# mlhenderson/cori-intml-examples

Hardware: AMD Instinct MI355X
Metric: images/sec (whole node) RPV CNN training (higher is better)
Workload: dtype bf16; 1 GPU; model=RPV CNN conv[16,32,64] fc[128] 64x64x3 (DistTrain_rpv), global_batch=128, per_gpu_batch=128, optimizer=Adam, parallelism=dp1, steps_per_graph=32

## Files before the change

### cori_intml_examples_amd/csrc/kernels/args.h

```cpp
#pragma once
#include "common.h"

struct BwdThrough {
  const bf16* prev_out = nullptr;
  const uint8_t* prev_code = nullptr;
  int prev_relu = 0, prev_pool = 0;
  int pH = 1, pW = 1, pC = 0, pCs = 0;
  int cH = 1, cW = 1;
  uint32_t drop_thr = 0;
  float drop_scale = 1.f;
  uint32_t seed = 0, stream_id = 0;
  bf16* dy = nullptr;
  int wt = 0;
};

struct PackRoute {
  int lo, hi, kind;
  int KHW, Cin, Cout, Cs, Csb;
  int NT, NTb;
  long long fwd, bwd;
};
#define MAX_ROUTES 8

struct OptimArgs {
// ... 145 lines not shown
  int spec = 1;
  int fix = 1;
};

struct WgradArgs {
  const bf16* x = nullptr;
  int B = 0, H = 0, W = 0, Cs_in = 0;
  int Ho = 0, Wo = 0, KH = 1, KW = 1, stride = 1, pad_t = 0, pad_l = 0;
  int Ktiles = 0;
  const bf16* dy = nullptr;
  int Cs_dy = 0;
  int NT = 0;
  int P = 0;
  int px_per_split = 0;
  int KT = 0;
  float* slab = nullptr;
  float* bslab = nullptr;
  int R = 1, blocks_per_split = 1;
  const uint8_t* dy_code = nullptr;
  int dHp = 0, dWp = 0;
  const bf16* zero = nullptr;
  int dbg = 0;
  unsigned long long* ts = nullptr;
  unsigned long long* ts2 = nullptr;
  OptimArgs opt;
  int opt_w = -1, opt_b = -1;
  int opt_nograd = 0;
  int spec = 1;
  long long pk_fwd = -1, pk_bwd = -1;
  int pk_NT = 0, pk_NTb = 0;
  int wt = 0;
  int xpix = 0, xrow = 0, dyld = 0;
  int kperm = 0;
  const int* xidx = nullptr;
  const StepState* xst = nullptr;
};

#define WG_GEO_INTS(F)                                                                                       \
  F(H) F(W) F(Cs_in) F(Ho) F(Wo) F(KH) F(KW) F(stride) F(pad_t) F(pad_l) F(Ktiles) F(NT) F(Cs_dy) F(dHp) F(dWp) \
  F(R) F(xpix) F(xrow) F(dyld) F(kperm) F(wt)

struct StepBeginArgs {
  StepState* st = nullptr;
  int training = 1;
  int bs = 0;
  int opt_kind = 0;
  float beta1 = 0.9f, beta2 = 0.999f, decay = 0.f, schedule_decay = 0.004f;
};

struct DenseFwdArgs {
  const bf16* x = nullptr;
  int M = 0, Ks = 0;
  const bf16* wpk = nullptr;
  int NT = 0, KS = 0;
  int splits = 1, ks_per_split = 0;
  float* part = nullptr;
  int mode = 0;
  const StepState* st = nullptr;
  BwdThrough bt;
  int book = 0;
  StepBeginArgs sb;
};

struct DenseEpiArgs {
  const float* part = nullptr;
  int splits = 1, M = 0, N = 0, Ns = 0, ldp = 0;
  const float* bias = nullptr;
  int relu = 0;
  bf16* out = nullptr;
// ... 246 lines not shown
```

### cori_intml_examples_amd/csrc/kernels/bindings.cpp

```cpp
#include <algorithm>
#include <pybind11/pybind11.h>
#include <pybind11/stl.h>

#include "args.h"

namespace py = pybind11;

void launch_conv_halo(const ConvMMArgs& a, int ntc, hipStream_t s);
size_t conv_halo_lds_bytes(const ConvMMArgs& a, int ntc);
void launch_conv_tile(const ConvMMArgs& a, int ntc, hipStream_t s, bool big, int nbuf);
bool launch_conv_hs(const ConvMMArgs& a, int ntc, hipStream_t s, int nwv, int order);
bool conv_hs_ok(const ConvMMArgs& a, int ntc, int nwv);
long long conv_tile_big_blocks(const ConvMMArgs& a, int ntc);
size_t conv_tile_lds_bytes(int ntc);
void launch_wgrad_tile(const WgradArgs& a, int ntc, hipStream_t s);
size_t wgrad_tile_lds_bytes(int ntc);
void launch_wgrad_halo(const WgradArgs& a, int MT, int NTT, int splits, hipStream_t s);
size_t wgrad_halo_lds_bytes(const WgradArgs& a, int MT, int NTT);
int wgrad_halo_resident(const WgradArgs& a, int MT, int NTT, bool bias);
int wgrad_halo_variant(const WgradArgs& a, int MT, int NTT);
int dual_halo_variant(const ConvMMArgs& ca, int ntc, const WgradArgs& wa, int MT, int NTT, bool xp, bool extras);
bool dual_halo_dgrad_fixed(const ConvMMArgs& ca, int ntc, const WgradArgs& wa, int MT, int NTT, bool xp, bool extras);
int head_rows_per_block(bool fused);
int head_epi_max();
void launch_wgrad(const WgradArgs& a, int ktw, int ntt, int splits, hipStream_t s);
size_t wgrad_lds_bytes(int KT, int NTT);
void launch_dense_fwd(const DenseFwdArgs& a, hipStream_t s);
void launch_dense_epi(const DenseEpiArgs& a, hipStream_t s);
int dense_groups(int M, int NT, int KS);
bool dense_big(int NT, int KS);
void launch_head(const HeadArgs& a, hipStream_t s);
bool launch_dual_halo(const ConvMMArgs& ca, int ntc, const WgradArgs& wa, int MT, int NTT, int splits,
                      const DualExtra& x, hipStream_t s);
bool launch_dense_bwd_dual(const WgradArgs& wa, int ktw, int ntt, int splits, const DenseFwdArgs& da,
                           hipStream_t s);
void launch_dense_wgrad(const WgradArgs& a, int kg, int ntt, int splits, hipStream_t s, int order, bool late);
size_t dense_wgrad_lds_bytes(int kg, int ntt);
void launch_dense_dx(const DenseFwdArgs& a, int ntc, hipStream_t s);
void launch_dense_bwd_pair(const WgradArgs& wa, int kg, int ntt, int splits, const DenseFwdArgs& da, int ntc,
                           hipStream_t s);
void launch_conv_stack_fwd(const ConvStackArgs& a, hipStream_t s);
void launch_init_params(const InitArgs& a, hipStream_t s);
void launch_synth(const SynthArgs& a, hipStream_t s);
int conv_stack_threads();
int conv_stack_variant(const ConvStackArgs& a);
bool conv_stack_fixed(const ConvStackArgs& a);
int conv_stack_tabn();
void launch_prologue(const PrologueArgs& a, const PackTable& tab, hipStream_t s);
int gather_gx(int R);
void launch_slab_reduce(float* grad, int lo, int hi, const RedTable& tab, hipStream_t s);
void launch_reduce_optim_end(float* grad, const RedTable& tc, const OptimArgs& a, const XgmiPush& xc,
                             const RedTable& te, const XgmiPush& xe, hipStream_t s);
void launch_reduce_optim(float* grad, const RedTable& tab, const OptimArgs& a, hipStream_t s,
                         const XgmiPush* xp = nullptr);
void launch_optim(const OptimArgs& a, const PackTable& tab, hipStream_t s);
// ... 67 lines not shown
  m.doc() = "cori_intml_examples_amd gfx950 HIP kernels";

  py::class_<BwdThrough>(m, "BwdThrough")
      .def(py::init<>())
      PTR(BwdThrough, prev_out) PTR(BwdThrough, prev_code) RW(BwdThrough, prev_relu)
      RW(BwdThrough, prev_pool) RW(BwdThrough, pH) RW(BwdThrough, pW) RW(BwdThrough, pC)
      RW(BwdThrough, pCs) RW(BwdThrough, cH) RW(BwdThrough, cW) RW(BwdThrough, drop_thr)
      RW(BwdThrough, drop_scale) RW(BwdThrough, seed) RW(BwdThrough, stream_id) PTR(BwdThrough, dy) RW(BwdThrough, wt);

  py::class_<ConvMMArgs>(m, "ConvMMArgs")
      .def(py::init<>())
      PTR(ConvMMArgs, x) RW(ConvMMArgs, B) RW(ConvMMArgs, H) RW(ConvMMArgs, W) RW(ConvMMArgs, Cs_in)
      RW(ConvMMArgs, Ho) RW(ConvMMArgs, Wo) RW(ConvMMArgs, KH) RW(ConvMMArgs, KW) RW(ConvMMArgs, stride)
      RW(ConvMMArgs, pad_t) RW(ConvMMArgs, pad_l) RW(ConvMMArgs, in_dil) RW(ConvMMArgs, KS)
      PTR(ConvMMArgs, wpk) RW(ConvMMArgs, NT) PTR(ConvMMArgs, bias) RW(ConvMMArgs, N) RW(ConvMMArgs, mode)
      RW(ConvMMArgs, flat_out) RW(ConvMMArgs, relu) RW(ConvMMArgs, pool) PTR(ConvMMArgs, out)
      RW(ConvMMArgs, Cs_out) RW(ConvMMArgs, Hp) RW(ConvMMArgs, Wp) PTR(ConvMMArgs, code)
      RW(ConvMMArgs, drop_thr) RW(ConvMMArgs, drop_scale) RW(ConvMMArgs, seed) RW(ConvMMArgs, stream_id)
      PTR(ConvMMArgs, st) RW(ConvMMArgs, bt) RW(ConvMMArgs, R) PTR(ConvMMArgs, in_code) PTR(ConvMMArgs, zero)
      RW(ConvMMArgs, in_pH) RW(ConvMMArgs, in_pW) RW(ConvMMArgs, dbg) PTR(ConvMMArgs, ts) RW(ConvMMArgs, xpix) RW(ConvMMArgs, kpipe) RW(ConvMMArgs, tm)
      RW(ConvMMArgs, spec);

  py::class_<WgradArgs>(m, "WgradArgs")
      .def(py::init<>())
      PTR(WgradArgs, x) RW(WgradArgs, B) RW(WgradArgs, H) RW(WgradArgs, W) RW(WgradArgs, Cs_in)
      RW(WgradArgs, Ho) RW(WgradArgs, Wo) RW(WgradArgs, KH) RW(WgradArgs, KW) RW(WgradArgs, stride)
      RW(WgradArgs, pad_t) RW(WgradArgs, pad_l) RW(WgradArgs, Ktiles) PTR(WgradArgs, dy)
      RW(WgradArgs, Cs_dy) RW(WgradArgs, NT) RW(WgradArgs, P) RW(WgradArgs, px_per_split)
      RW(WgradArgs, KT) PTR(WgradArgs, slab) PTR(WgradArgs, bslab) RW(WgradArgs, R)
      RW(WgradArgs, blocks_per_split) PTR(WgradArgs, dy_code) PTR(WgradArgs, zero) RW(WgradArgs, dHp) RW(WgradArgs, dWp)
      RW(WgradArgs, dbg) PTR(WgradArgs, ts) PTR(WgradArgs, ts2) RW(WgradArgs, opt) RW(WgradArgs, opt_w)
      RW(WgradArgs, opt_b) RW(WgradArgs, xpix) RW(WgradArgs, xrow) RW(WgradArgs, dyld) RW(WgradArgs, kperm)
      PTR(WgradArgs, xidx) PTR(WgradArgs, xst) RW(WgradArgs, pk_fwd) RW(WgradArgs, pk_bwd) RW(WgradArgs, pk_NT)
      RW(WgradArgs, pk_NTb) RW(WgradArgs, wt) RW(WgradArgs, opt_nograd) RW(WgradArgs, spec);

  py::class_<DenseFwdArgs>(m, "DenseFwdArgs")
      .def(py::init<>())
      PTR(DenseFwdArgs, x) RW(DenseFwdArgs, M) RW(DenseFwdArgs, Ks) PTR(DenseFwdArgs, wpk)
      RW(DenseFwdArgs, NT) RW(DenseFwdArgs, KS) RW(DenseFwdArgs, splits) RW(DenseFwdArgs, ks_per_split)
      PTR(DenseFwdArgs, part) RW(DenseFwdArgs, mode) PTR(DenseFwdArgs, st) RW(DenseFwdArgs, bt)
      RW(DenseFwdArgs, book) RW(DenseFwdArgs, sb);

  py::class_<DenseEpiArgs>(m, "DenseEpiArgs")
      .def(py::init<>())
      PTR(DenseEpiArgs, part) RW(DenseEpiArgs, splits) RW(DenseEpiArgs, M) RW(DenseEpiArgs, N)
      RW(DenseEpiArgs, Ns) RW(DenseEpiArgs, ldp) PTR(DenseEpiArgs, bias) RW(DenseEpiArgs, relu)
      PTR(DenseEpiArgs, out) RW(DenseEpiArgs, drop_thr) RW(DenseEpiArgs, drop_scale)
      RW(DenseEpiArgs, seed) RW(DenseEpiArgs, stream_id) PTR(DenseEpiArgs, st);

  py::class_<HeadArgs>(m, "HeadArgs")
      .def(py::init<>())
      PTR(HeadArgs, h) RW(HeadArgs, M) RW(HeadArgs, K) RW(HeadArgs, Ks) RW(HeadArgs, N)
      RW(HeadArgs, flat_C) RW(HeadArgs, flat_Cs) PTR(HeadArgs, w) PTR(HeadArgs, bias) PTR(HeadArgs, y)
      RW(HeadArgs, act) RW(HeadArgs, training) RW(HeadArgs, inv_bs) PTR(HeadArgs, st) PTR(HeadArgs, probs)
      PTR(HeadArgs, wslab) PTR(HeadArgs, bslab) RW(HeadArgs, bt) RW(HeadArgs, epi) PTR(HeadArgs, ts)
      PTR(HeadArgs, yidx) RW(HeadArgs, generic) PTR(HeadArgs, wb);


  py::class_<GatherArgs>(m, "GatherArgs")
      .def(py::init<>())
      PTR(GatherArgs, xs) PTR(GatherArgs, ys) PTR(GatherArgs, perm) PTR(GatherArgs, st)
      RW(GatherArgs, bs) RW(GatherArgs, R) RW(GatherArgs, C) RW(GatherArgs, Nd) PTR(GatherArgs, xb)
      PTR(GatherArgs, yb) RW(GatherArgs, skip_x) PTR(GatherArgs, wb);

  py::class_<StepBeginArgs>(m, "StepBeginArgs")
      .def(py::init<>())
      PTR(StepBeginArgs, st) RW(StepBeginArgs, training) RW(StepBeginArgs, bs) RW(StepBeginArgs, opt_kind)
// ... 141 lines not shown
        const int epb = d.vec4 ? 1024 / d.tpe : 256 / d.tpe;
        t.nblocks += (numel + epb - 1) / epb;
      }, py::arg("slab"), py::arg("stride_s"), py::arg("S"), py::arg("ld"), py::arg("dst_off"), py::arg("numel"),
      py::arg("type"), py::arg("KH"), py::arg("KW"), py::arg("Cin"), py::arg("Cout"), py::arg("Cs"), py::arg("tpe") = -1);

  m.attr("STEP_STATE_BYTES") = (int)sizeof(StepState);
  m.def("set_red_lanes", [](int n) {
    if (n < 1 || n > 256) throw std::invalid_argument("red_lanes: 1..256");
    g_red_lanes = n;
  });
  static_assert(sizeof(PackRoute) == 56 && offsetof(PackRoute, fwd) == 40, "PackRoute layout (models/plan routes)");
  m.attr("PACK_ROUTE_BYTES") = (int)sizeof(PackRoute);
  m.attr("MAX_ROUTES") = MAX_ROUTES;
  m.attr("MAX_RED") = MAX_RED;
  m.attr("STEP_STATE_METRICS_OFFSET") = (int)offsetof(StepState, metric_slots);
  m.attr("STEP_STATE_METRIC_SLOTS") = 16;
  m.attr("STEP_STATE_MSCHED_OFFSET") = (int)offsetof(StepState, m_schedule);
  m.attr("STEP_STATE_LR_OFFSET") = (int)offsetof(StepState, lr);
  m.attr("STEP_STATE_S_OFFSET") = (int)offsetof(StepState, s);
  m.attr("STEP_STATE_WARM_OFFSET") = (int)offsetof(StepState, warm_t0);
  m.attr("STEP_STATE_DATA_OFFSET") = (int)offsetof(StepState, data_x);
  m.attr("STEP_STATE_DATAN_OFFSET") = (int)offsetof(StepState, data_n);
  m.attr("STEP_STATE_DATAW_OFFSET") = (int)offsetof(StepState, data_w);

  m.def("wgrad_lds_bytes", &wgrad_lds_bytes);
  m.def("conv_halo_lds_bytes", &conv_halo_lds_bytes);
  m.def("wgrad_halo_lds_bytes", &wgrad_halo_lds_bytes);
  m.def("wgrad_halo_resident", &wgrad_halo_resident);
  m.def("wgrad_halo_variant", &wgrad_halo_variant);
  m.def("dual_halo_variant", &dual_halo_variant, py::arg("ca"), py::arg("ntc"), py::arg("wa"), py::arg("MT"),
        py::arg("NTT"), py::arg("xp") = false, py::arg("extras") = false);
  m.def("dual_halo_dgrad_fixed", &dual_halo_dgrad_fixed, py::arg("ca"), py::arg("ntc"), py::arg("wa"), py::arg("MT"),
        py::arg("NTT"), py::arg("xp") = false, py::arg("extras") = false);
  m.def("head_rows_per_block", &head_rows_per_block, py::arg("fused") = false);
  m.def("conv_tile_lds_bytes", &conv_tile_lds_bytes);
  m.def("conv_tile", [](const ConvMMArgs& a, int ntc, uintptr_t s, bool big, int nbuf) {
    launch_conv_tile(a, ntc, S(s), big, nbuf); check_last("conv_tile"); }, py::arg("a"), py::arg("ntc"), py::arg("s"),
    py::arg("big") = false, py::arg("nbuf") = 4);
  m.def("conv_tile_big_blocks", &conv_tile_big_blocks);
  m.def("conv_hs_ok", &conv_hs_ok, py::arg("a"), py::arg("ntc"), py::arg("nwv") = 8);
  m.def("conv_hs", [](const ConvMMArgs& a, int ntc, uintptr_t s, int nwv, int order) {
    const bool ok = launch_conv_hs(a, ntc, S(s), nwv, order); check_last("conv_hs"); return ok; },
    py::arg("a"), py::arg("ntc"), py::arg("s"), py::arg("nwv") = 8, py::arg("order") = 0,
    "halo-staged wide conv (stride 1 or the parity classes of a strided dgrad, whole-row blocks of "
    "32 * nwv rows); false (nothing launched) for other shapes");
  m.def("wgrad_tile_lds_bytes", &wgrad_tile_lds_bytes);
  m.def("wgrad_tile", [](const WgradArgs& a, int ntc, uintptr_t s) {
    launch_wgrad_tile(a, ntc, S(s)); check_last("wgrad_tile"); });
  m.def("conv_halo", [](const ConvMMArgs& a, int ntc, uintptr_t s) {
    launch_conv_halo(a, ntc, S(s)); check_last("conv_halo"); });
  m.def("wgrad_halo", [](const WgradArgs& a, int MT, int NTT, int splits, uintptr_t s) {
    launch_wgrad_halo(a, MT, NTT, splits, S(s)); check_last("wgrad_halo"); });
  m.def("wgrad", [](const WgradArgs& a, int ktw, int ntt, int splits, uintptr_t s) {
    launch_wgrad(a, ktw, ntt, splits, S(s)); check_last("wgrad"); });
  m.def("dense_fwd", [](const DenseFwdArgs& a, uintptr_t s) { launch_dense_fwd(a, S(s)); check_last("dense_fwd"); });
  m.def("dense_groups", &dense_groups, "work items per K-split of dense_fwd for (M, NT, KS)");
  m.def("dense_big", &dense_big, "dense_fwd uses the large-weight LDS path for (NT, KS)");
  m.def("dense_epi", [](const DenseEpiArgs& a, uintptr_t s) { launch_dense_epi(a, S(s)); check_last("dense_epi"); });
  m.def("head", [](const HeadArgs& a, uintptr_t s) { launch_head(a, S(s)); check_last("head"); });
  m.def("prologue", [](const PrologueArgs& a, const PackTable& t, uintptr_t s) {
    launch_prologue(a, t, S(s)); check_last("prologue"); });
  m.def("gather_gx", &gather_gx);
  m.def("head_epi_max", &head_epi_max);
  m.def("reduce_optim_end", [](uintptr_t grad, const RedTable& tc, const OptimArgs& a, uintptr_t s,
                               const XgmiPush& xc, const RedTable& te, const XgmiPush& xe) {
    if (!xc.on || !xe.on || xc.mode != 3 || xe.mode != 5) throw std::invalid_argument("reduce_optim_end: modes 3 + 5");
// ... 224 lines not shown
```

### cori_intml_examples_amd/csrc/kernels/wgrad_halo.hip

```cpp

#include <algorithm>
#include <cstdlib>

#include "wgrad_halo_body.h"
#include "wgrad_sig.h"

template <int MTW, int NTT, bool CS4, bool PIPE, bool INSTR>
__global__ __launch_bounds__(256) void wgrad_halo_kernel(const WgradArgs a, const int MT) {
  extern __shared__ __attribute__((aligned(16))) char smem[];
  const size_t lin = blockIdx.x + (size_t)gridDim.x * (blockIdx.y + (size_t)gridDim.y * blockIdx.z);
  if (INSTR && a.ts && threadIdx.x == 0) a.ts[2 * lin] = wall_clock64();
  wgrad_halo_body<MTW, NTT, CS4, PIPE, INSTR>(a, MT, blockIdx.x, blockIdx.y, blockIdx.z, smem);
  if (INSTR && a.ts) {
    __syncthreads();
    if (threadIdx.x == 0) a.ts[2 * lin + 1] = wall_clock64();
  }
}

static bool wh_instr(const WgradArgs& a) { return a.dbg || a.ts || a.ts2; }

size_t wgrad_halo_lds_bytes(const WgradArgs& a, int MT, int NTT) {
  const int W_in = (a.Wo - 1) * a.stride + a.KW;
  const int R_in = (a.R - 1) * a.stride + a.KH;
  const int XP = a.xpix ? a.xpix : a.Cs_in, XR = a.xrow ? a.xrow : W_in;
  const int ldb = a.dyld ? a.dyld : NTT * 16 + 8;
  const size_t x_elems = (size_t)(((R_in * XR * XP) + 7) & ~7);
  const size_t npb32 = (size_t)((a.R * a.Wo + 31) & ~31);
  return std::max<size_t>(x_elems * 2 + npb32 * ldb * 2 + 128 + (size_t)(MT * 4 + 4) * 4, 4 * 16 * WH_SQ * 4);
}

template <int MTW, int NTT, bool CS4>
static void wh_t(const WgradArgs& a, int MT, dim3 grid, size_t lds, hipStream_t s) {
  const bool pipe = grid.x * grid.y * grid.z < 512 && a.blocks_per_split > 1;
  auto k = wh_instr(a) ? (pipe ? wgrad_halo_kernel<MTW, NTT, CS4, true, true> : wgrad_halo_kernel<MTW, NTT, CS4, false, true>)
                       : (pipe ? wgrad_halo_kernel<MTW, NTT, CS4, true, false> : wgrad_halo_kernel<MTW, NTT, CS4, false, false>);
  if (lds > 65536) (void)hipFuncSetAttribute((const void*)k, hipFuncAttributeMaxDynamicSharedMemorySize, (int)lds);
  hipLaunchKernelGGL(k, grid, dim3(256), lds, s, a, MT);
}

int wgrad_halo_variant(const WgradArgs& a, int MT, int NTT) {
  if (!a.spec || wh_instr(a)) return 0;
  const int v = wgrad_sig_find(a, MT, NTT);
  return v && wgrad_sig_at(v).alone ? v : 0;
}

void launch_wgrad_halo(const WgradArgs& a, int MT, int NTT, int splits, hipStream_t s) {
  const bool cs4 = a.Cs_in == 4;
  dim3 grid(splits, (a.NT + NTT - 1) / NTT, (a.Ktiles + MT - 1) / MT);
  const size_t lds = wgrad_halo_lds_bytes(a, MT, NTT);
  if (const int v = wgrad_halo_variant(a, MT, NTT)) {
    wgrad_sig_at(v).alone(a, grid, lds, grid.x * grid.y * grid.z < 512 && a.blocks_per_split > 1, s);
    return;
  }
  const int mtw = (MT + (a.bslab ? 1 : 0) + 3) / 4;
#define C(M_, N_)                                            \
  if (mtw <= M_ && NTT == N_) {                              \
    if (cs4) wh_t<M_, N_, true>(a, MT, grid, lds, s);     \
    else wh_t<M_, N_, false>(a, MT, grid, lds, s);        \
    return;                                                  \
  }
  C(1, 1) C(2, 1) C(4, 1) C(1, 2) C(2, 2) C(4, 2) C(1, 4) C(2, 4) C(4, 4) C(1, 8) C(2, 8)
#undef C
}

int wgrad_halo_resident(const WgradArgs& a, int MT, int NTT, bool bias) {
  const bool cs4 = a.Cs_in == 4;
  const size_t lds = wgrad_halo_lds_bytes(a, MT, NTT);
  const int mtw = (MT + (bias ? 1 : 0) + 3) / 4;
  const void* k = nullptr;
  const bool in = wh_instr(a);
#define C(M_, N_)                                                                                       \
  if (!k && mtw <= M_ && NTT == N_)                                                                     \
    k = cs4 ? (in ? (const void*)wgrad_halo_kernel<M_, N_, true, false, true>                           \
                  : (const void*)wgrad_halo_kernel<M_, N_, true, false, false>)                         \
            : (in ? (const void*)wgrad_halo_kernel<M_, N_, false, false, true>                          \
                  : (const void*)wgrad_halo_kernel<M_, N_, false, false, false>);
  C(1, 1) C(2, 1) C(4, 1) C(1, 2) C(2, 2) C(4, 2) C(1, 4) C(2, 4) C(4, 4) C(1, 8) C(2, 8)
#undef C
  if (!k) return 0;
  int dev = 0, per_cu = 0;
  hipDeviceProp_t prop;
  if (hipGetDevice(&dev) != hipSuccess || hipGetDeviceProperties(&prop, dev) != hipSuccess) return 0;
  if (lds > 65536) (void)hipFuncSetAttribute(k, hipFuncAttributeMaxDynamicSharedMemorySize, (int)lds);
  if (hipOccupancyMaxActiveBlocksPerMultiprocessor(&per_cu, k, 256, lds) != hipSuccess) return 0;
// ... 3 lines not shown
```

### cori_intml_examples_amd/csrc/kernels/wgrad_halo_body.h

```cpp
#pragma once
#include "bwd_through.h"

struct XChunk4 { bf16x4 v; int o; };
struct XChunk8 { bf16x8 v; int o; };

__device__ __forceinline__ bf16x4 tr_read_h(const bf16* p) {
  return __builtin_amdgcn_ds_read_tr16_b64_v4bf16(LDS_PTR(bf16x4, p));
}

#define WH_STAMP(i)                                                                     \
  if (INSTR && a.ts2 && threadIdx.x == 0 && (i) < 16) a.ts2[(size_t)blockIdx.x * 16 + (i)] = wall_clock64();

struct WgGeoRt {
#define F(n) \
  __device__ __forceinline__ static int n(const WgradArgs& a) { return a.n; }
  WG_GEO_INTS(F)
#undef F
  __device__ __forceinline__ static int MT(int mt_launch) { return mt_launch; }
  __device__ __forceinline__ static bool pooled(const WgradArgs& a) { return a.dy_code != nullptr; }
  __device__ __forceinline__ static bool bias(const WgradArgs& a) { return a.bslab != nullptr; }
  __device__ __forceinline__ static bool xidx(const WgradArgs& a) { return a.xidx != nullptr; }
};
template <class S, bool XIDX>
struct WgGeoFix {
#define F(n) \
  __device__ __forceinline__ static constexpr int n(const WgradArgs&) { return S::n; }
  WG_GEO_INTS(F)
#undef F
  __device__ __forceinline__ static constexpr int MT(int) { return S::MT; }
  __device__ __forceinline__ static constexpr bool pooled(const WgradArgs&) { return S::pooled; }
  __device__ __forceinline__ static constexpr bool bias(const WgradArgs&) { return S::bias; }
  __device__ __forceinline__ static constexpr bool xidx(const WgradArgs&) { return XIDX; }
};

template <class G>
__device__ __forceinline__ const bf16* wg_xbase(const WgradArgs& a, int b) {
  if (G::xidx(a)) return reinterpret_cast<const bf16*>(a.xst->data_x) + (size_t)a.xidx[b] * a.xst->data_R;
  return a.x + (size_t)b * G::H(a) * G::W(a) * G::Cs_in(a);
}

#define WH_SQ 20

template <int MTW, int NTT, bool CS4, bool PIPE, bool INSTR = true, class G = WgGeoRt>
__device__ __forceinline__ void wgrad_halo_body(const WgradArgs& a, const int MT_launch, const int bx, const int by,
                                                const int bz, char* smem) {
  const int MT = G::MT(MT_launch);
  const int dbg = INSTR ? a.dbg : 0;
  const int R = G::R(a), s = G::stride(a), Cs = G::Cs_in(a);
  const int W_in = (G::Wo(a) - 1) * s + G::KW(a);
  const int R_in = (R - 1) * s + G::KH(a);
  const int npb = R * G::Wo(a);
  const int npb32 = (npb + 31) & ~31;
  const int XP = G::xpix(a) ? G::xpix(a) : Cs, XR = G::xrow(a) ? G::xrow(a) : W_in;
  const int ldb = G::dyld(a) ? G::dyld(a) : NTT * 16 + 8;
  bf16* xl = reinterpret_cast<bf16*>(smem);
  const int x_elems = ((R_in * XR * XP) + 7) & ~7;
  bf16* dyl = xl + x_elems;
  bf16* zl = dyl + (size_t)npb32 * ldb;
  bf16* ol = zl + 32;
  int* ktab = reinterpret_cast<int*>(zl + 64);

  const int tid = threadIdx.x, wave = __builtin_amdgcn_readfirstlane(tid >> 6), lane = tid & 63, i = lane & 15,
            g = lane >> 4;
  const int mt0 = bz * MT;
  const int nt0 = by * NTT;
  const int KHW = G::KH(a) * G::KW(a);
  const bool do_bias = G::bias(a) && bz == 0;
  const int MTb = MT + (do_bias ? 1 : 0);

  WH_STAMP(0);
  if (tid < 32) reinterpret_cast<uint32_t*>(zl)[tid] = tid < 16 ? 0u : 0x3F803F80u;
  for (int c = tid; c < MT * 4; c += 256) {
    const int k = (mt0 + c / 4) * 16 + 4 * (c & 3);
    const int tap = k / Cs;
    int e = -1;
    if (tap < KHW && mt0 + c / 4 < G::Ktiles(a)) {
// ... 101 lines not shown
          off0 = ((y0 * s) * XR + (q0 - y0 * G::Wo(a)) * s) * XP;
          off1 = ((y1 * s) * XR + (q1 - y1 * G::Wo(a)) * s) * XP;
        }
        const bf16* pbrow = dyl + (size_t)P0 * ldb + 4 * (i & 3);
  #pragma unroll
        for (int v = 0; v < NTT; ++v) {
          const bf16* pb = pbrow + v * 16;
          bfr[v] = __builtin_shufflevector(tr_read_h(pb), tr_read_h(pb + (P1 - P0) * ldb), 0, 1, 2, 3, 4, 5, 6, 7);
        }
  #pragma unroll
        for (int u = 0; u < MTW; ++u) {
          const bf16* pz = u == ubias ? ol : zl;
          const bf16* pa0 = ko[u] >= 0 ? xl + off0 + ko[u] : pz;
          const bf16* pa1 = ko[u] >= 0 ? xl + off1 + ko[u] : pz;
          afr[u] = __builtin_shufflevector(tr_read_h(pa0), tr_read_h(pa1), 0, 1, 2, 3, 4, 5, 6, 7);
        }
      };
      auto mmas = [&](const bf16x8 (&afr)[MTW], const bf16x8 (&bfr)[NTT]) {
  #pragma unroll
        for (int u = 0; u < MTW; ++u)
          if (u < nval) {
  #pragma unroll
            for (int v = 0; v < NTT; ++v) acc[u][v] = mfma16(afr[u], bfr[v], acc[u][v]);
          }
      };
      for (int ks = 0; ks < nks; ++ks) {
        bf16x8 bfr[NTT], afr[MTW];
        frags(ks, afr, bfr);
        mmas(afr, bfr);
      }
  };

  constexpr int WH_PX = 4, WH_PY = 4;
  if (PIPE && dbg_stage && nch_x <= WH_PX * 256 && (pexp ? nq : nch_y) <= WH_PY * 256) {
    uint4 xr[WH_PX], yr[WH_PY];
    int xa[WH_PX];
    uint2 yc[WH_PY];
    uint32_t yp[WH_PY];
    int xrow[WH_PX], xoff[WH_PX], qoff[WH_PY], qdst[WH_PY];
    uint32_t xcol = 0;
#pragma unroll
    for (int u = 0; u < WH_PX; ++u) {
      const int idx = min(tid + u * 256, nch_x - 1);
      const int pix = fcpp.div(idx), c = (idx - pix * cpp) * cw;
      const int r = fwin.div(pix), px = pix - r * W_in;
      const int ix = px - G::pad_l(a);
      xa[u] = (r * XR + px) * XP + c;
      xrow[u] = r;
      xoff[u] = (r * G::W(a) + ix) * Cs + c;
      if (ix >= 0 && ix < G::W(a)) xcol |= 1u << u;
    }
    if (pexp) {
#pragma unroll
      for (int u = 0; u < WH_PY; ++u) {
        const int q = min(tid + u * 256, nq - 1);
        const int p2 = fcpr.div(q), ch = q - p2 * cpr;
        const int ry = fhw.div(p2), wx = p2 - ry * hw;
        qoff[u] = (ry * G::dWp(a) + wx) * G::Cs_dy(a) + nt0 * 16 + ch * 8;
        qdst[u] = ((2 * ry) * G::Wo(a) + 2 * wx) * ldb + ch * 8;
      }
    }
    auto fetch = [&](const int blk) {
      const int b = blk / nrb, oy0 = (blk - b * nrb) * R;
      const int npix = min(R, G::Ho(a) - oy0) * G::Wo(a);
      const int yb = oy0 * s - G::pad_t(a);
      const bf16* xbase = wg_xbase<G>(a, b);
// ... 227 lines not shown
```

### cori_intml_examples_amd/csrc/kernels/wgrad_sig.h

```cpp
#pragma once
#include <hip/hip_runtime.h>

#include <type_traits>

#include "args.h"

#define WG_SIG_INTS(F) WG_GEO_INTS(F) F(MT) F(NTT)

#define WG_SIG(NAME, H_, W_, CS_, HO_, WO_, PAD_, KT_, NT_, CSDY_, DHP_, DWP_, POOLED_, R_, XPIX_, XROW_, DYLD_, MT_, \
               NTT_)                                                                                                 \
  struct NAME {                                                                                                      \
    static constexpr int H = H_, W = W_, Cs_in = CS_, Ho = HO_, Wo = WO_, KH = 3, KW = 3, stride = 1, pad_t = PAD_,  \
                         pad_l = PAD_, Ktiles = KT_, NT = NT_, Cs_dy = CSDY_, dHp = DHP_, dWp = DWP_, R = R_,        \
                         xpix = XPIX_, xrow = XROW_, dyld = DYLD_, kperm = 1, wt = 1, MT = MT_, NTT = NTT_;          \
    static constexpr bool pooled = POOLED_, bias = true;                                                             \
                                           \
    static constexpr int MTW = (MT_ + 1 + 3) / 4 <= 1 ? 1 : ((MT_ + 1 + 3) / 4 <= 2 ? 2 : 4);                        \
  }

WG_SIG(WgSigRpv1, 64, 64, 4, 64, 64, 1, 3, 1, 16, 32, 32, true, 8, 4, 74, 16, 3, 1);
WG_SIG(WgSigRpv2, 32, 32, 16, 32, 32, 1, 9, 2, 32, 16, 16, true, 8, 16, 34, 48, 9, 2);
WG_SIG(WgSigRpv3, 16, 16, 32, 16, 16, 1, 18, 4, 64, 8, 8, true, 8, 48, 18, 80, 9, 4);
WG_SIG(WgSigMnist1, 28, 28, 4, 26, 26, 0, 3, 2, 32, 0, 0, false, 8, 4, 42, 48, 3, 2);
WG_SIG(WgSigMnist2, 26, 26, 32, 24, 24, 0, 18, 4, 64, 12, 12, true, 5, 48, 26, 80, 9, 4);
// ... 40 lines not shown
constexpr WgSigVals wg_sig_vals() {
  return WgSigVals{
#define F(n) S::n,
      WG_SIG_INTS(F)
#undef F
          S::pooled ? 1 : 0,
      S::bias ? 1 : 0};
}

typedef void (*WgSigLaunch)(const WgradArgs& a, dim3 grid, size_t lds, bool pipe, hipStream_t s);
typedef void (*DualSigLaunch)(const ConvMMArgs& ca, const WgradArgs& wa, dim3 wg, int cgx, int cgy, size_t lds,
                              const DualExtra& x, hipStream_t s);
#define DUAL_SIG_DECL(NAME)                                                                                  \
  void NAME(const ConvMMArgs& ca, const WgradArgs& wa, dim3 wg, int cgx, int cgy, size_t lds, const DualExtra& x, \
            hipStream_t s)
DUAL_SIG_DECL(dual_sig_rpv2_tm1);
DUAL_SIG_DECL(dual_sig_rpv2_tm4);
DUAL_SIG_DECL(dual_sig_rpv3_tm1);
DUAL_SIG_DECL(dual_sig_rpv3_tm4);
DUAL_SIG_DECL(dual_sig_mnist2_tm1);
DUAL_SIG_DECL(dual_sig_mnist2_tm2);
DUAL_SIG_DECL(dual_fix_rpv2_tm4);
DUAL_SIG_DECL(dual_fix_rpv3_tm4);
DUAL_SIG_DECL(dual_fix_mnist2_tm2);

struct WgradSig {
  WgSigVals v;
  WgSigLaunch alone;
  DualSigLaunch dual[3];
  DgSigVals dg;
  DualSigLaunch fix;
};

int wgrad_sig_find(const WgradArgs& a, int MT, int NTT);
const WgradSig& wgrad_sig_at(int v);
bool dgrad_sig_matches(const ConvMMArgs& a, int ntc, int tm, int v);
```

### cori_intml_examples_amd/csrc/kernels/wgrad_sig.hip

```cpp
#include "wgrad_halo_sig_body.h"

template <class SIG>
static void wgrad_sig_launch(const WgradArgs& a, dim3 grid, size_t lds, bool pipe, hipStream_t s) {
  void (*k)(const WgradArgs) =
      a.xidx ? (pipe ? wgrad_halo_sig_kernel<SIG, true, true> : wgrad_halo_sig_kernel<SIG, false, true>)
             : (pipe ? wgrad_halo_sig_kernel<SIG, true, false> : wgrad_halo_sig_kernel<SIG, false, false>);
  if (lds > 65536) (void)hipFuncSetAttribute((const void*)k, hipFuncAttributeMaxDynamicSharedMemorySize, (int)lds);
  hipLaunchKernelGGL(k, grid, dim3(256), lds, s, a);
}

static const WgradSig kWgradSigs[] = {
    {wg_sig_vals<WgSigRpv1>(), wgrad_sig_launch<WgSigRpv1>, {nullptr, nullptr, nullptr}, {}, nullptr},
    {wg_sig_vals<WgSigRpv2>(), nullptr, {dual_sig_rpv2_tm1, nullptr, dual_sig_rpv2_tm4},
     dg_sig_vals<DgSigRpv2>(), dual_fix_rpv2_tm4},
    {wg_sig_vals<WgSigRpv3>(), nullptr, {dual_sig_rpv3_tm1, nullptr, dual_sig_rpv3_tm4},
     dg_sig_vals<DgSigRpv3>(), dual_fix_rpv3_tm4},
    {wg_sig_vals<WgSigMnist1>(), wgrad_sig_launch<WgSigMnist1>, {nullptr, nullptr, nullptr}, {}, nullptr},
    {wg_sig_vals<WgSigMnist2>(), nullptr, {dual_sig_mnist2_tm1, dual_sig_mnist2_tm2, nullptr},
     dg_sig_vals<DgSigMnist2>(), dual_fix_mnist2_tm2},
};
static_assert(std::is_same<DgSigRpv2::Wg, WgSigRpv2>::value && std::is_same<DgSigRpv3::Wg, WgSigRpv3>::value &&
                  std::is_same<DgSigMnist2::Wg, WgSigMnist2>::value,
              "a table row pairs a wgrad signature with its own layer's dgrad");

static bool wg_sig_matches(const WgradArgs& a, int MT, int NTT, const WgSigVals& v) {
  if ((a.dy_code != nullptr) != (v.pooled != 0) || (a.bslab != nullptr) != (v.bias != 0)) return false;
  if (MT != v.MT || NTT != v.NTT) return false;
  WgSigVals w = v;
#define F(n) w.n = a.n;
  WG_GEO_INTS(F)
#undef F
  if (!v.pooled) w.dHp = v.dHp, w.dWp = v.dWp;
#define F(n) \
  if (w.n != v.n) return false;
  WG_GEO_INTS(F)
#undef F
  return true;
}

int wgrad_sig_find(const WgradArgs& a, int MT, int NTT) {
  const int nsig = (int)(sizeof(kWgradSigs) / sizeof(kWgradSigs[0]));
  for (int i = 0; i < nsig; ++i)
    if (wg_sig_matches(a, MT, NTT, kWgradSigs[i].v)) return i + 1;
  return 0;
}

const WgradSig& wgrad_sig_at(int v) { return kWgradSigs[v - 1]; }

bool dgrad_sig_matches(const ConvMMArgs& a, int ntc, int tm, int v) {
  const DgSigVals& d = kWgradSigs[v - 1].dg;
  if (!kWgradSigs[v - 1].fix || !d.TM || tm != d.TM || ntc != 1 || a.mode != 1) return false;
  if ((a.in_code != nullptr) != (d.pooled != 0)) return false;
#define F(n) \
  if (a.n != d.n) return false;
  CV_GEO_INTS(F)
#undef F
// ... 7 lines not shown
```

### cori_intml_examples_amd/models/hip_geometry.py

```python
from __future__ import annotations

from typing import NamedTuple, Optional

import torch

from ..utils.tune import tune
from . import lds_layout
from .step_program import cdiv, dropout_pair


def _pow2_le(x, cap):
    p = 1
    while p * 2 <= min(x, cap):
        p *= 2
    return p


class Wgrad(NamedTuple):
    a: object
    tiles: tuple
    splits: int
    slab: Optional[torch.Tensor]
    bslab: Optional[torch.Tensor]

# ... 319 lines not shown

        def fits(r):
            w_in = (g.Wo - 1) * g.stride + g.KW
            nch_x = ((r - 1) * g.stride + g.KH) * w_in * cpp
            nch_y = cdiv(r * g.Wo, 32) * 32 * NTT * 2
            return nch_x <= 1024 and nch_y <= 1024
        for r in range(R, 0, -1):
            if fits(r) or not tune("wgrad_fit", layer=g.i):
                R = r
                break
        a.kperm = int(tune("wgrad_perm")) | (0 if tune("wgrad_fast") else 2)
        if tune("lds_layout"):
            a.xpix, a.xrow, a.dyld = lds_layout.wgrad_layout(g.Cs_in, W_in, g.Wo, NTT, g.KH, g.KW, g.stride,
                                                             a.Ktiles, bool(a.kperm & 1))
        XP, XR = (a.xpix or g.Cs_in), (a.xrow or W_in)
        while R > 1 and (((R - 1) * g.stride + g.KH) * XR * XP * 2 > 64 * 1024):
            R -= 1
        a.R = R
        nblocks = bs * cdiv(g.Ho, R)
        groups = cdiv(NT, NTT) * cdiv(a.Ktiles, MT)
        per_split_bytes = a.Ktiles * 16 * NT * 16 * 4
        s_budget = max(1, (tune("wgrad_slab_mb") << 20) // per_split_bytes)
        cap = tune("wgrad_splits", layer=g.i) or K.wgrad_halo_resident(a, MT, NTT, bool(bias)) or 768
        S = max(1, min(nblocks, s_budget, max(1, cap // groups)))
        bps = cdiv(nblocks, S)
        S = cdiv(nblocks, bps)
        a.blocks_per_split = bps
        lds = K.wgrad_halo_lds_bytes(a, MT, NTT)
        if lds > 150 * 1024:
            raise NotImplementedError("wgrad halo stage too large (%d bytes)" % lds)
        slab, bslab = self._wgrad_slabs(a, S, bias)
        a.wt = int(bool(int(tune("wt")) & 4) and slab.numel() * 4 < (1 << 31))
        a.spec = int(tune("wgrad_spec"))
        return Wgrad(a, (MT, NTT), S, slab, bslab)

    def _wgrad_args(self, xin, width, dy, Cs_dy, N, bias, direct=None):
        if not (width == 4 or width % 8 == 0):
            raise NotImplementedError("wgrad needs Cs_in == 4 or a multiple of 8 (got %d)" % width)
        NT = cdiv(N, 16)
        a = self._wgrad_base(xin, 1, 1, width, 1, 1, (1, 1, 1, 0, 0), dy, Cs_dy, NT)
        P = a.P
        ntt = _pow2_le(NT, 8)
        ktw = 4 if ntt <= 4 else 2
        while ktw > 1 and 4 * (ktw // 2) >= a.Ktiles:
            ktw //= 2
        if ntt == 8 and ktw == 4:
            ktw = 2
        a.KT = 4 * ktw
        gy = cdiv(a.Ktiles, a.KT)
        gz = cdiv(NT, ntt)
        per_split_bytes = a.Ktiles * 16 * NT * 16 * 4
        s_budget = max(1, (4 << 20) // per_split_bytes)
        S = 1 if direct else max(1, min(512 // max(1, gy * gz), s_budget, cdiv(P, 32)))
        pps = cdiv(cdiv(P, S), 32) * 32
        S = cdiv(P, pps)
        a.px_per_split = pps
        return Wgrad(a, (ktw, ntt), S, *self._wgrad_slabs(a, S, bias, direct))

    def _dense_wgrad_args(self, xin, width, dh, Ns, N, bias, direct=None):
        bs, NT = self.bs, cdiv(N, 16)
        a = self._wgrad_base(xin, 1, 1, width, 1, 1, None, dh, Ns, NT)
        ntt = _pow2_le(NT, min(8, tune("dw_ntt")))
        kg = 2
        groups = cdiv(a.Ktiles, kg) * cdiv(NT, ntt)
        per_split_bytes = a.Ktiles * 16 * NT * 16 * 4
        s_budget = max(1, (tune("dw_slab_mb") << 20) // per_split_bytes)
# ... 19 lines not shown
```

### cori_intml_examples_amd/utils/tune.py

```python
from __future__ import annotations

import difflib
import os
from typing import Dict, NamedTuple, Optional, Tuple

EXACT = "exact"
PATH = "path"
ABLATION = "ablation"
KINDS = (EXACT, PATH, ABLATION)

LAYER, LAYER_ONLY = "layer", "layer_only"


class Knob(NamedTuple):
    key: str
    default: object
    kind: str
    doc: str
    per_layer: str = ""
    auto: bool = False
    layer_defaults: Optional[Dict[int, object]] = None

    def parse(self, v: str):
        d = self.default
# ... 56 lines not shown
    Knob("dgrad_ntc", 1, PATH, "n-tiles per workgroup of a co-scheduled dgrad (1: each workgroup stages "
         "half the weights, the launch fits the CUs in one wave)"),
    Knob("dgrad_tm", 0, PATH, "co-scheduled dgrad m-tiles per wave per pass of conv layer <i>; 0 = the "
         "kernel's choice", per_layer=LAYER_ONLY, auto=True),
    Knob("dgrad_dbg", 0, EXACT, "ConvMMArgs::dbg A/B switches of the dgrad (exact ones only; 32: no "
         "one-batch prologue, test_dgrad_onebatch_prologue_bit_identical)"),
    Knob("wgrad_tile_ntc", 0, PATH, "cap on the n-tiles per block of the tiled (wide conv) wgrad; "
         "0 = auto: 8 / 4 / 2 by the layer's n-tiles", auto=True),
    Knob("wgrad_tile_fill", 1, PATH, "tiled wgrad split count: this many rounds of resident workgroups "
         "(two per CU), never one workgroup more (legacy conv3 wgrad 113 us at 486 workgroups, 185 us "
         "at 522; profiles/r6_wgrad_splits_ab.txt)"),
    Knob("wgrad_tile_wgs", 0, PATH, "tiled wgrad workgroups wanted; 0 = auto: wgrad_tile_fill rounds",
         auto=True),
    Knob("wgrad_tile_slab_mb", 64, PATH, "byte budget (MiB) of the tiled wgrad's partial slabs"),
    Knob("wgrad_block_px", 256, PATH, "pixels per block of the halo wgrad (first layer, a standalone "
         "launch: 512 = 8 RPV rows, +0.2-0.5 %, profiles/r4m_ab_rpv.txt, r4n_ab_rpv.txt)",
         per_layer=LAYER, layer_defaults={0: 512}),
    Knob("wgrad_max_rows", 8, PATH, "most rows per block of the halo wgrad", per_layer=LAYER),
    Knob("wgrad_fit", True, PATH, "conv layer <i>: prefer the largest block whose staging fits the halo "
         "wgrad's register pipeline (wgrad_halo_body.h WH_PX / WH_PY)", per_layer=LAYER_ONLY),
    Knob("wgrad_perm", True, PATH, "WgradArgs::kperm bit 0: the halo wgrad's k index <-> pixel permutation "
         "within a 32-pixel k-step" + _NO_EVIDENCE),
    Knob("wgrad_fast", True, PATH, "0 sets WgradArgs::kperm bit 1: the halo wgrad without its "
         "row-aligned fast path" + _NO_EVIDENCE),
    Knob("wgrad_slab_mb", 8, PATH, "byte budget (MiB) of a halo wgrad's partial slabs"),
    Knob("wgrad_splits", 0, PATH, "halo wgrad workgroups across its splits; 0 = auto: one round of "
         "resident workgroups (the generic instance's occupancy x CUs); changes the summation order "
         "(profiles/r2_v12_wgrad_split_sweep.txt)", per_layer=LAYER, auto=True),
    Knob("wgrad_spec", 1, EXACT, "layer-signature halo wgrad instances (csrc/kernels/wgrad_sig.h) where "
         "one matches; 0: always the generic kernels (tests/test_wgrad_sig.py)"),
    Knob("dgrad_spec", 1, EXACT, "dual launches whose co-scheduled dgrad geometry is fixed at compile time "
         "too (csrc/kernels/dual_halo_fix_body.h) where the dgrad signature matches; 0: the dual launch "
         "as without it (tests/test_dgrad_sig.py)"),
    Knob("dense_big_wgs", 256, PATH, "workgroups wanted for a large dense layer's forward (one per CU)"),
    Knob("dense_big_minks", 8, PATH, "fewest k-steps per split of a large dense layer's forward"),
    Knob("dense_waves", 2048, PATH, "16x16-tile waves wanted for a small dense layer's split-K forward"),
    Knob("dense_bwd2", True, PATH, "dense_bwd.hip kernels (per-wave pipelined wgrad, vectorised dX "
         "epilogue) where their 8-element alignment holds; 0: generic wgrad / split-K"),
    Knob("dual_dense", True, PATH, "one launch for a dense layer's wgrad and dX" + _NO_EVIDENCE),
    Knob("dw_ntt", 4, PATH, "most n-tiles per workgroup of dense_wgrad (4: twice the workgroups of 8 -- "
         "RPV +0.6 %, MNIST +1.2 %, profiles/r4s_ab_rpv.txt, r4s_ab_mnist.txt)"),
    Knob("dw_slab_mb", 8, PATH, "byte budget (MiB) of dense_wgrad's partial slabs"),
    Knob("dw_min_wgs", 256, PATH, "workgroups wanted for dense_wgrad (sets its batch splits)"),
    Knob("dw_order", 1, PATH, "dense_wgrad grid order; 1: the n groups of one feature group consecutive "
         "(legacy -5 us, profiles/r6_dense_wgrad_ab.txt)" + _NO_EVIDENCE),
    Knob("dw_late", True, PATH, "dense_wgrad at 4 waves / SIMD (legacy 1.070 -> 1.059 ms)" + _NO_EVIDENCE),
    Knob("dx_ntc", 0, PATH, "n-tiles per wave of dense_dx (1, 2, 4; test_dense_dx_tiles_agree); 0 = auto: "
         "the most that leaves dx_min_wgs workgroups", auto=True),
    Knob("dx_min_wgs", 256, PATH, "fewest workgroups of dense_dx (256: the RPV dense dX at 2 n-tiles per "
         "wave, 3 us faster than 512 one-tile workgroups, profiles/r4p_ab_rpv.txt)"),
    Knob("dense_opt", "auto", PATH, "the optimizer update inside the one-split dense wgrad: auto = only "
         "layers whose gradient is written in place (> 16 MB; legacy 1.269 -> 1.238 ms/step, "
         "profiles/r4c_ab_legacy.txt), truthy = every one-split layer, falsy = off "
         "(tests/test_dense_bwd.py)"),
    Knob("opt_nograd", True, PATH, "a dense wgrad with the fused update does not store the gradient it "
         "consumed (profiles/r6_dense_wgrad_ab.txt); 0 keeps it readable through the store"
         + _NO_EVIDENCE),
    Knob("fuse_head", True, PATH, "the head launch runs the last dense layer's split-K epilogue; same "
         "activations, the loss metric differs in fp32 rounding (tests/test_head_edges.py)"),
    Knob("head_generic", False, EXACT, "1: the head kernel without its fast paths "
         "(test_head_fast_paths_bit_identical)"),
    Knob("red_lanes", 16, PATH, "slab partials per reduction split-lane (set_red_lanes); changes the "
         "summation order"),
    Knob("red_desc_max", 16, PATH, "most descriptors of the ONE end-of-step reduction table (RedTable "
         "capacity, MAX_RED); more: 1 MiB buckets and a separate optimizer launch"),
    Knob("fuse_optim", True, PATH, "the Keras update fused into the reduction launch (and, with "
# ... 127 lines not shown
```

Measured before the change: 1.719 million images/s.

## Add depth-two software-pipelined staging for the RPV first-layer halo wgrad

New measurement: 1.770 million images/s, median of 6. 1.03x the previous value.

```diff
diff --git a/cori_intml_examples_amd/csrc/kernels/args.h b/cori_intml_examples_amd/csrc/kernels/args.h
--- a/cori_intml_examples_amd/csrc/kernels/args.h
+++ b/cori_intml_examples_amd/csrc/kernels/args.h
@@ -201,9 +201,12 @@
   int wt = 0;
   int xpix = 0, xrow = 0, dyld = 0;
   int kperm = 0;
+  int depth = 0;
   const int* xidx = nullptr;
   const StepState* xst = nullptr;
 };
+static_assert(offsetof(WgradArgs, xidx) == offsetof(WgradArgs, depth) + 4 && offsetof(WgradArgs, depth) % 8 == 4,
+              "WgradArgs::depth fills padding: no kernel argument moves");
 
 #define WG_GEO_INTS(F)                                                                                       \
   F(H) F(W) F(Cs_in) F(Ho) F(Wo) F(KH) F(KW) F(stride) F(pad_t) F(pad_l) F(Ktiles) F(NT) F(Cs_dy) F(dHp) F(dWp) \
diff --git a/cori_intml_examples_amd/csrc/kernels/bindings.cpp b/cori_intml_examples_amd/csrc/kernels/bindings.cpp
--- a/cori_intml_examples_amd/csrc/kernels/bindings.cpp
+++ b/cori_intml_examples_amd/csrc/kernels/bindings.cpp
@@ -21,6 +21,7 @@
 int wgrad_halo_variant(const WgradArgs& a, int MT, int NTT);
 int dual_halo_variant(const ConvMMArgs& ca, int ntc, const WgradArgs& wa, int MT, int NTT, bool xp, bool extras);
 bool dual_halo_dgrad_fixed(const ConvMMArgs& ca, int ntc, const WgradArgs& wa, int MT, int NTT, bool xp, bool extras);
+int wgrad_halo_depth(const WgradArgs& a, int MT, int NTT, int splits);
 int head_rows_per_block(bool fused);
 int head_epi_max();
 void launch_wgrad(const WgradArgs& a, int ktw, int ntt, int splits, hipStream_t s);
@@ -154,7 +155,8 @@
       RW(WgradArgs, dbg) PTR(WgradArgs, ts) PTR(WgradArgs, ts2) RW(WgradArgs, opt) RW(WgradArgs, opt_w)
       RW(WgradArgs, opt_b) RW(WgradArgs, xpix) RW(WgradArgs, xrow) RW(WgradArgs, dyld) RW(WgradArgs, kperm)
       PTR(WgradArgs, xidx) PTR(WgradArgs, xst) RW(WgradArgs, pk_fwd) RW(WgradArgs, pk_bwd) RW(WgradArgs, pk_NT)
-      RW(WgradArgs, pk_NTb) RW(WgradArgs, wt) RW(WgradArgs, opt_nograd) RW(WgradArgs, spec);
+      RW(WgradArgs, pk_NTb) RW(WgradArgs, wt) RW(WgradArgs, opt_nograd) RW(WgradArgs, spec)
+      RW(WgradArgs, depth);
 
   py::class_<DenseFwdArgs>(m, "DenseFwdArgs")
       .def(py::init<>())
@@ -362,6 +364,7 @@
         py::arg("NTT"), py::arg("xp") = false, py::arg("extras") = false);
   m.def("dual_halo_dgrad_fixed", &dual_halo_dgrad_fixed, py::arg("ca"), py::arg("ntc"), py::arg("wa"), py::arg("MT"),
         py::arg("NTT"), py::arg("xp") = false, py::arg("extras") = false);
+  m.def("wgrad_depth_variant", &wgrad_halo_depth, py::arg("wa"), py::arg("MT"), py::arg("NTT"), py::arg("splits"));
   m.def("head_rows_per_block", &head_rows_per_block, py::arg("fused") = false);
   m.def("conv_tile_lds_bytes", &conv_tile_lds_bytes);
   m.def("conv_tile", [](const ConvMMArgs& a, int ntc, uintptr_t s, bool big, int nbuf) {
diff --git a/cori_intml_examples_amd/csrc/kernels/wgrad_deep.hip b/cori_intml_examples_amd/csrc/kernels/wgrad_deep.hip
--- /dev/null
+++ b/cori_intml_examples_amd/csrc/kernels/wgrad_deep.hip
@@ -0,0 +1,20 @@
+#include "wgrad_halo_sig_body.h"
+
+template <class SIG, bool XIDX, int DEPTH>
+__global__ __launch_bounds__(256) void wgrad_halo_deep_kernel(const WgradArgs a) {
+  extern __shared__ __attribute__((aligned(16))) char smem[];
+  static_assert(SIG::Cs_in == 4 && DEPTH > 1, "standalone signature instances are the 4-channel first layers");
+  wgrad_halo_body<SIG::MTW, SIG::NTT, true, true, false, WgGeoFix<SIG, XIDX>, DEPTH>(a, SIG::MT, blockIdx.x,
+                                                                                    blockIdx.y, blockIdx.z, smem);
+}
+
+template <class SIG, int DEPTH>
+static void wgrad_deep_launch(const WgradArgs& a, dim3 grid, size_t lds, hipStream_t s) {
+  void (*k)(const WgradArgs) = a.xidx ? wgrad_halo_deep_kernel<SIG, true, DEPTH> : wgrad_halo_deep_kernel<SIG, false, DEPTH>;
+  if (lds > 65536) (void)hipFuncSetAttribute((const void*)k, hipFuncAttributeMaxDynamicSharedMemorySize, (int)lds);
+  hipLaunchKernelGGL(k, grid, dim3(256), lds, s, a);
+}
+
+void wgrad_deep_rpv1(const WgradArgs& a, dim3 grid, size_t lds, hipStream_t s) {
+  wgrad_deep_launch<WgSigRpv1, 2>(a, grid, lds, s);
+}
diff --git a/cori_intml_examples_amd/csrc/kernels/wgrad_halo.hip b/cori_intml_examples_amd/csrc/kernels/wgrad_halo.hip
--- a/cori_intml_examples_amd/csrc/kernels/wgrad_halo.hip
+++ b/cori_intml_examples_amd/csrc/kernels/wgrad_halo.hip
@@ -44,12 +44,25 @@
   return v && wgrad_sig_at(v).alone ? v : 0;
 }
 
+static dim3 wh_grid(const WgradArgs& a, int MT, int NTT, int splits) {
+  return dim3(splits, (a.NT + NTT - 1) / NTT, (a.Ktiles + MT - 1) / MT);
+}
+static bool wh_pipe(const WgradArgs& a, dim3 grid) { return grid.x * grid.y * grid.z < 512 && a.blocks_per_split > 1; }
+
+int wgrad_halo_depth(const WgradArgs& a, int MT, int NTT, int splits) {
+  const int v = wgrad_halo_variant(a, MT, NTT);
+  if (!v || wh_pipe(a, wh_grid(a, MT, NTT, splits))) return 1;
+  const WgradDeep& dp = wgrad_deep_at(v);
+  return dp.alone && (a.depth == 0 || a.depth == dp.depth) ? dp.depth : 1;
+}
+
 void launch_wgrad_halo(const WgradArgs& a, int MT, int NTT, int splits, hipStream_t s) {
   const bool cs4 = a.Cs_in == 4;
-  dim3 grid(splits, (a.NT + NTT - 1) / NTT, (a.Ktiles + MT - 1) / MT);
+  const dim3 grid = wh_grid(a, MT, NTT, splits);
   const size_t lds = wgrad_halo_lds_bytes(a, MT, NTT);
   if (const int v = wgrad_halo_variant(a, MT, NTT)) {
-    wgrad_sig_at(v).alone(a, grid, lds, grid.x * grid.y * grid.z < 512 && a.blocks_per_split > 1, s);
+    if (wgrad_halo_depth(a, MT, NTT, splits) > 1) wgrad_deep_at(v).alone(a, grid, lds, s);
+    else wgrad_sig_at(v).alone(a, grid, lds, wh_pipe(a, grid), s);
     return;
   }
   const int mtw = (MT + (a.bslab ? 1 : 0) + 3) / 4;
diff --git a/cori_intml_examples_amd/csrc/kernels/wgrad_halo_body.h b/cori_intml_examples_amd/csrc/kernels/wgrad_halo_body.h
--- a/cori_intml_examples_amd/csrc/kernels/wgrad_halo_body.h
+++ b/cori_intml_examples_amd/csrc/kernels/wgrad_halo_body.h
@@ -1,4 +1,6 @@
 #pragma once
+#include <type_traits>
+
 #include "bwd_through.h"
 
 struct XChunk4 { bf16x4 v; int o; };
@@ -20,6 +22,7 @@
   __device__ __forceinline__ static bool pooled(const WgradArgs& a) { return a.dy_code != nullptr; }
   __device__ __forceinline__ static bool bias(const WgradArgs& a) { return a.bslab != nullptr; }
   __device__ __forceinline__ static bool xidx(const WgradArgs& a) { return a.xidx != nullptr; }
+  static constexpr bool fixed = false;
 };
 template <class S, bool XIDX>
 struct WgGeoFix {
@@ -31,6 +34,8 @@
   __device__ __forceinline__ static constexpr bool pooled(const WgradArgs&) { return S::pooled; }
   __device__ __forceinline__ static constexpr bool bias(const WgradArgs&) { return S::bias; }
   __device__ __forceinline__ static constexpr bool xidx(const WgradArgs&) { return XIDX; }
+  static constexpr bool fixed = true;
+  using Sig = S;
 };
 
 template <class G>
@@ -41,7 +46,7 @@
 
 #define WH_SQ 20
 
-template <int MTW, int NTT, bool CS4, bool PIPE, bool INSTR = true, class G = WgGeoRt>
+template <int MTW, int NTT, bool CS4, bool PIPE, bool INSTR = true, class G = WgGeoRt, int DEPTH = 1>
 __device__ __forceinline__ void wgrad_halo_body(const WgradArgs& a, const int MT_launch, const int bx, const int by,
                                                 const int bz, char* smem) {
   const int MT = G::MT(MT_launch);
@@ -209,6 +214,92 @@
   };
 
   constexpr int WH_PX = 4, WH_PY = 4;
+  if constexpr (DEPTH > 1) {
+    static_assert(PIPE && !INSTR && G::fixed, "the deep pipeline is built for production signature instances");
+    using S = typename G::Sig;
+    constexpr int c_Rin = (S::R - 1) * S::stride + S::KH, c_Win = (S::Wo - 1) * S::stride + S::KW;
+    constexpr int NX = (c_Rin * c_Win * (S::Cs_in / (CS4 ? 4 : 8)) + 255) / 256;
+    constexpr int NY = ((S::R >> 1) * (S::Wo >> 1) * NTT * 2 + 255) / 256;
+    static_assert(S::pooled && (S::R & 1) == 0 && S::Ho % S::R == 0 && (S::Wo & 1) == 0 && ((S::R * S::Wo) & 31) == 0 &&
+                      S::NT % NTT == 0 && S::NT * 16 <= S::Cs_dy && 2 * S::dHp >= S::Ho && 2 * S::dWp >= S::Wo,
+                  "a deep stage holds pooled dY chunks (pexp)");
+    static_assert(NX <= WH_PX && NY <= WH_PY, "one block's staging fits the pipeline's chunk budget");
+    using XT = typename std::conditional<CS4, uint2, uint4>::type;
+    struct Stage {
+      XT xr[NX];
+      uint4 yr[NY];
+      uint2 yc[NY];
+    };
+    Stage st[DEPTH];
+    int xa[NX], xrow[NX], xoff[NX], qoff[NY], qdst[NY];
+    uint32_t xcol = 0;
+#pragma unroll
+    for (int u = 0; u < NX; ++u) {
+      const int idx = min(tid + u * 256, nch_x - 1);
+      const int pix = fcpp.div(idx), c = (idx - pix * cpp) * cw;
+      const int r = fwin.div(pix), px = pix - r * W_in;
+      const int ix = px - G::pad_l(a);
+      xa[u] = (r * XR + px) * XP + c;
+      xrow[u] = r;
+      xoff[u] = (r * G::W(a) + ix) * Cs + c;
+      if (ix >= 0 && ix < G::W(a)) xcol |= 1u << u;
+    }
+#pragma unroll
+    for (int u = 0; u < NY; ++u) {
+      const int q = min(tid + u * 256, nq - 1);
+      const int p2 = fcpr.div(q), ch = q - p2 * cpr;
+      const int ry = fhw.div(p2), wx = p2 - ry * hw;
+      qoff[u] = (ry * G::dWp(a) + wx) * G::Cs_dy(a) + nt0 * 16 + ch * 8;
+      qdst[u] = ((2 * ry) * G::Wo(a) + 2 * wx) * ldb + ch * 8;
+    }
+    auto x_ok = [&](const int u, const int blk) {
+      const int b = blk / nrb, iy = (blk - b * nrb) * R * s - G::pad_t(a) + xrow[u];
+      return ((xcol >> u) & 1u) && iy >= 0 && iy < G::H(a);
+    };
+    auto fetch = [&](Stage& t, const int blk) {
+      const int b = blk / nrb, oy0 = (blk - b * nrb) * R;
+      const bf16* xbase = wg_xbase<G>(a, b);
+      const bf16* xrow0 = xbase + (ptrdiff_t)(oy0 * s - G::pad_t(a)) * G::W(a) * Cs;
+#pragma unroll
+      for (int u = 0; u < NX; ++u) t.xr[u] = *reinterpret_cast<const XT*>(x_ok(u, blk) ? xrow0 + xoff[u] : xbase);
+      const size_t qb = (((size_t)b * G::dHp(a) + (oy0 >> 1)) * G::dWp(a)) * G::Cs_dy(a);
+#pragma unroll
+      for (int u = 0; u < NY; ++u) {
+        const size_t o = qb + qoff[u];
+        t.yr[u] = *reinterpret_cast<const uint4*>(a.dy + o);
+        t.yc[u] = *reinterpret_cast<const uint2*>(a.dy_code + o);
+      }
+    };
+    auto commit = [&](const Stage& t, const int blk) {
+#pragma unroll
+      for (int u = 0; u < NX; ++u) {
+        const bool ok = x_ok(u, blk);
+        XT v = t.xr[u];
+        v.x = ok ? v.x : 0u, v.y = ok ? v.y : 0u;
+        if constexpr (!CS4) v.z = ok ? v.z : 0u, v.w = ok ? v.w : 0u;
+        *reinterpret_cast<XT*>(xl + xa[u]) = v;
+      }
+#pragma unroll
+      for (int u = 0; u < NY; ++u) pq_store_at(qdst[u], t.yr[u], t.yc[u]);
+    };
+#pragma unroll
+    for (int d = 0; d < DEPTH; ++d) {
+      fetch(st[d], min(blk0 + d, blk1 - 1));
+      __builtin_amdgcn_sched_barrier(0);
+    }
+    for (int blk = blk0;;) {
+#pragma unroll
+      for (int d = 0; d < DEPTH; ++d, ++blk) {
+        if (blk >= blk1) goto deep_done;
+        if (blk != blk0) __syncthreads();
+        commit(st[d], blk);
+        __syncthreads();
+        fetch(st[d], min(blk + DEPTH, blk1 - 1));
+        mma_block(npb);
+      }
+    }
+  deep_done:;
+  } else
   if (PIPE && dbg_stage && nch_x <= WH_PX * 256 && (pexp ? nq : nch_y) <= WH_PY * 256) {
     uint4 xr[WH_PX], yr[WH_PY];
     int xa[WH_PX];
diff --git a/cori_intml_examples_amd/csrc/kernels/wgrad_sig.h b/cori_intml_examples_amd/csrc/kernels/wgrad_sig.h
--- a/cori_intml_examples_amd/csrc/kernels/wgrad_sig.h
+++ b/cori_intml_examples_amd/csrc/kernels/wgrad_sig.h
@@ -96,6 +96,15 @@
   DualSigLaunch fix;
 };
 
+typedef void (*WgDeepLaunch)(const WgradArgs& a, dim3 grid, size_t lds, hipStream_t s);
+void wgrad_deep_rpv1(const WgradArgs& a, dim3 grid, size_t lds, hipStream_t s);
+
+struct WgradDeep {
+  int depth;
+  WgDeepLaunch alone;
+};
+const WgradDeep& wgrad_deep_at(int v);
+
 int wgrad_sig_find(const WgradArgs& a, int MT, int NTT);
 const WgradSig& wgrad_sig_at(int v);
 bool dgrad_sig_matches(const ConvMMArgs& a, int ntc, int tm, int v);
diff --git a/cori_intml_examples_amd/csrc/kernels/wgrad_sig.hip b/cori_intml_examples_amd/csrc/kernels/wgrad_sig.hip
--- a/cori_intml_examples_amd/csrc/kernels/wgrad_sig.hip
+++ b/cori_intml_examples_amd/csrc/kernels/wgrad_sig.hip
@@ -22,6 +22,14 @@
 static_assert(std::is_same<DgSigRpv2::Wg, WgSigRpv2>::value && std::is_same<DgSigRpv3::Wg, WgSigRpv3>::value &&
                   std::is_same<DgSigMnist2::Wg, WgSigMnist2>::value,
               "a table row pairs a wgrad signature with its own layer's dgrad");
+
+static const WgradDeep kWgradDeep[] = {
+    {2, wgrad_deep_rpv1}, {1, nullptr}, {1, nullptr}, {1, nullptr}, {1, nullptr},
+};
+static_assert(sizeof(kWgradDeep) / sizeof(kWgradDeep[0]) == sizeof(kWgradSigs) / sizeof(kWgradSigs[0]),
+              "a deep row per signature");
+
+const WgradDeep& wgrad_deep_at(int v) { return kWgradDeep[v - 1]; }
 
 static bool wg_sig_matches(const WgradArgs& a, int MT, int NTT, const WgSigVals& v) {
   if ((a.dy_code != nullptr) != (v.pooled != 0) || (a.bslab != nullptr) != (v.bias != 0)) return false;
diff --git a/cori_intml_examples_amd/models/hip_geometry.py b/cori_intml_examples_amd/models/hip_geometry.py
--- a/cori_intml_examples_amd/models/hip_geometry.py
+++ b/cori_intml_examples_amd/models/hip_geometry.py
@@ -375,6 +375,7 @@
         slab, bslab = self._wgrad_slabs(a, S, bias)
         a.wt = int(bool(int(tune("wt")) & 4) and slab.numel() * 4 < (1 << 31))
         a.spec = int(tune("wgrad_spec"))
+        a.depth = int(tune("wgrad_depth"))
         return Wgrad(a, (MT, NTT), S, slab, bslab)
 
     def _wgrad_args(self, xin, width, dy, Cs_dy, N, bias, direct=None):
diff --git a/cori_intml_examples_amd/utils/tune.py b/cori_intml_examples_amd/utils/tune.py
--- a/cori_intml_examples_amd/utils/tune.py
+++ b/cori_intml_examples_amd/utils/tune.py
@@ -112,6 +112,10 @@
     Knob("dgrad_spec", 1, EXACT, "dual launches whose co-scheduled dgrad geometry is fixed at compile time "
          "too (csrc/kernels/dual_halo_fix_body.h) where the dgrad signature matches; 0: the dual launch "
          "as without it (tests/test_dgrad_sig.py)"),
+    Knob("wgrad_depth", 0, EXACT, "blocks of a halo wgrad split whose staging loads are in flight at once, in "
+         "the launches that have a deep instance (csrc/kernels/wgrad_deep.hip: the RPV first layer): 0 the "
+         "instance's own depth, 1 the depth-one kernels, d that depth where it is built "
+         "(profiles/wgrad_depth_ab.txt; tests/test_wgrad_depth.py)"),
     Knob("dense_big_wgs", 256, PATH, "workgroups wanted for a large dense layer's forward (one per CU)"),
     Knob("dense_big_minks", 8, PATH, "fewest k-steps per split of a large dense layer's forward"),
     Knob("dense_waves", 2048, PATH, "16x16-tile waves wanted for a small dense layer's split-K forward"),
```
